# zju3dv/street_gaussians

Hardware: AMD Instinct MI355X
Metric: train iters/s (fwd+bwd) @1M Gaussians 1920x1280 SH3 (higher is better)
Workload: dtype f32

## Files before the change

### street_gaussians_amd/csrc/sgr_blend_bwd.hip

```cpp
#include "sgr_math.h"
#include "sgr_reduce.h"

#include <type_traits>

#ifndef SGR_WITH_VARIANTS
#define SGR_WITH_VARIANTS 0
#endif

#define SGR_TILE_THREADS 256
typedef float sgr_f2 __attribute__((ext_vector_type(2)));
#ifndef SGR_BWD_BATCH
#define SGR_BWD_BATCH 128
#endif
#ifndef SGR_BWD_BATCH_WIDE
#define SGR_BWD_BATCH_WIDE 64
#endif
#ifndef SGR_BWD_WAVES
#define SGR_BWD_WAVES(SMAX) ((SMAX) >= 12 && (SMAX) <= 16 ? 6 : ((SMAX) >= 20 && (SMAX) <= 24 ? 5 : ((SMAX) > 24 ? 4 : 1)))
#endif
template <int SMAX>
struct SgrBwdBatch { static constexpr int value = SMAX <= 8 ? SGR_BWD_BATCH : SGR_BWD_BATCH_WIDE; };
#define SGR_ROW_BASE 11
#ifndef SGR_FACTORED
#define SGR_FACTORED 1
#endif
#ifndef SGR_EXACT_BWD_FAST
#define SGR_EXACT_BWD_FAST 1
#endif
#ifndef SGR_BWD_NEWTON
#define SGR_BWD_NEWTON 0
#endif
#ifndef SGR_EXACT_BWD_GUARD
#define SGR_EXACT_BWD_GUARD 1
#endif
#ifndef SGR_EXACT_TRIM
#define SGR_EXACT_TRIM 1
#endif
#ifndef SGR_FOLD
#define SGR_FOLD 1
#endif
#ifndef SGR_VROWS
#define SGR_VROWS 1
#endif
#ifndef SGR_SPARSE_K
#define SGR_SPARSE_K 9
#endif

__global__ void sgr_wave_sum_test_kernel(const float* in, float* out_dpp, float* out_shfl) {
    const float v = in[blockIdx.x * 64 + threadIdx.x];
    float a = v, a1 = 2.f * v, a2 = -v, a3 = v + 1.f;
    sgr_wave_sum4(a, a1, a2, a3);
    const float b = sgr_wave_sum_shfl(v);
    const float c = sgr_wave_sum_dpp(v);
    float x[12], r[3];
#pragma unroll
    for (int i = 0; i < 12; i++) x[i] = (float)(i + 1) * v;
    sgr_wave_reduce_scatter<12>(x, r);
    const int k = threadIdx.x >> 4;
    const int perm = (k == 1) ? 2 : ((k == 2) ? 1 : k);
    bool rs_ok = true;
#pragma unroll
    for (int t = 0; t < 3; t++) rs_ok = rs_ok && (r[t] == (float)(4 * t + perm + 1) * b);
    {
        float y[12], g[1];
#pragma unroll
        for (int i = 0; i < 12; i++) y[i] = (float)(i + 1) * v;
        sgr_wave_reduce_fold<12>(y, g);
        const int bank = (threadIdx.x >> 2) & 3, t0 = (0x3120 >> (bank * 4)) & 3;
        if (t0 < 3) rs_ok = rs_ok && (g[0] == (float)(4 * t0 + perm + 1) * b);
        float z[32], gz[2];
#pragma unroll
        for (int i = 0; i < 32; i++) z[i] = (float)(i + 1) * v;
        sgr_wave_reduce_fold<32>(z, gz);
#pragma unroll
        for (int i = 0; i < 2; i++) rs_ok = rs_ok && (gz[i] == (float)(4 * (4 * i + t0) + perm + 1) * b);
        float w[20], gw[2];
#pragma unroll
        for (int i = 0; i < 20; i++) w[i] = (float)(i + 1) * v;
        sgr_wave_reduce_fold<20>(w, gw);
#pragma unroll
        for (int i = 0; i < 2; i++)
            if (4 * i + t0 < 5) rs_ok = rs_ok && (gw[i] == (float)(4 * (4 * i + t0) + perm + 1) * b);
    }
    {
        float z[24], g0, g1;
#pragma unroll
        for (int i = 0; i < 24; i++) z[i] = (float)(i + 1) * v;
        sgr_wave_reduce_fold24(z, g0, g1);
        const int bank = (threadIdx.x >> 2) & 3, pb = (0x3120 >> (bank * 4)) & 3;
        rs_ok = rs_ok && (g0 == (float)(4 * pb + perm + 1) * b);
        if ((bank & 1) == 0) rs_ok = rs_ok && (g1 == (float)(16 + 4 * pb + perm + 1) * b);
    }
    rs_ok = __all(rs_ok);
    if (threadIdx.x == 63) {
        const bool ok = (a1 == 2.f * a) && (a2 == -a) && (a3 == a + 64.f) && (c == a) && rs_ok;
        out_dpp[blockIdx.x] = ok ? a : __builtin_nanf("");
        out_shfl[blockIdx.x] = b;
    }
}
void sgr_launch_wave_sum_test(const float* in, float* out_dpp, float* out_shfl, int nwaves, hipStream_t s) {
    sgr_wave_sum_test_kernel<<<nwaves, 64, 0, s>>>(in, out_dpp, out_shfl);
}

__device__ __forceinline__ void sgr_lds_barrier() {
    asm volatile("s_waitcnt lgkmcnt(0)" ::: "memory");
    __syncthreads();
}

__device__ __forceinline__ uint32_t sgr_lds_addr(const float* p) {
    return (uint32_t)(uintptr_t)(__attribute__((address_space(3))) const float*)p;
}
__device__ __forceinline__ int sgr_popc64(uint64_t m) {
    int r;
    asm("s_bcnt1_i32_b64 %0, %1" : "=s"(r) : "s"(m) : "scc");
    return r;
}

template <int SMAX, bool CULL, bool DPP, bool DET, int BATCH, bool EXACT = false>
__device__ __forceinline__ void
sgr_blend_bwd_body(const uint2* __restrict__ ranges, const uint32_t* __restrict__ point_list, int W, int H, int S,
                     int gx, int gy, const float* __restrict__ bg_color, const float4* __restrict__ rec,
                     const uint32_t* __restrict__ u0, const uint64_t* __restrict__ tmask, const float* __restrict__ semantics, const float* __restrict__ alphas,
                     const uint32_t* __restrict__ n_contrib, const uint8_t* __restrict__ hit4,
                     const float* __restrict__ dL_dpixels, const float* __restrict__ dL_dpixel_depths,
                     const float* __restrict__ dL_dalphas, const float* __restrict__ dL_dpixel_semantics,
                     float* __restrict__ partials, int row_stride, uint8_t* __restrict__ touched, uint32_t row_limit,
                     const uint32_t* __restrict__ hlist, const uint32_t* __restrict__ n_contrib_k, const uint32_t* __restrict__ hl_flag) {
#pragma clang fp contract(off)
    constexpr int NS = SMAX > 0 ? SMAX : 1;
    constexpr int NVAL = (SGR_ROW_BASE + SMAX + 3) / 4 * 4;
    constexpr int ACCW = NVAL + (((NVAL / 4) & 1) ? 0 : 4);
    __shared__ float4 sA[BATCH];
    __shared__ float4 sB[BATCH];
    __shared__ float4 sC[BATCH];
    __shared__ uint64_t sBits[4][4];
    __shared__ uint64_t sVis[4][4];
    __shared__ int sMax[4];
    constexpr int NROW = DET ? 2 : 1;
    constexpr bool VROWS = SGR_VROWS && DET && DPP && SGR_FOLD && SMAX == 0;
    constexpr int CAP = NROW * BATCH;
    constexpr int NCH = BATCH / 64;
    constexpr int SPK = (VROWS && SMAX == 0) ? SGR_SPARSE_K : 0;
    constexpr int XROWS = 4 * SPK;
    static_assert(SPK == 0 || ACCW == 12, "a stage entry is a row of 12 floats");
    static_assert(SPK <= 16, "add sparse cases");
    __shared__ __attribute__((aligned(16))) float sAcc[(CAP + XROWS) * ACCW];
    __shared__ __attribute__((aligned(16))) float sSem[SMAX > 0 ? BATCH * SMAX : 4];

    const int tid = threadIdx.x, lane = tid & 63, wave = tid >> 6;
    uint32_t tx, ty;
    if (!sgr_wg_tile(blockIdx.x, gx, gy, ranges, tx, ty)) return;
    const uint32_t tile = ty * (uint32_t)gx + tx;
    const uint32_t px = tx * SGR_BLOCK_X + (wave & 1) * 8 + (lane & 7);
    const uint32_t py = ty * SGR_BLOCK_Y + (wave >> 1) * 8 + (lane >> 3);
    const bool inside = px < (uint32_t)W && py < (uint32_t)H;
    const float pxf = (float)px, pyf = (float)py;
    const size_t pix_id = (size_t)W * py + px;
    const size_t plane = (size_t)H * W;
    const uint2 range = ranges[tile];

    const float T_final = inside ? (1.0f - alphas[pix_id]) : 0.0f;
    float T = T_final;
    const bool HL = SGR_HLIST && CULL && hit4 != nullptr && hlist != nullptr && hl_flag[0] != 0u;
    const int lastc = inside ? (int)(HL ? n_contrib_k : n_contrib)[pix_id] : 0;
    float dLdC0 = 0.f, dLdC1 = 0.f, dLdC2 = 0.f, dLdD = 0.f, dLdA = 0.f;
    float dLdS[NS];
#pragma unroll
    for (int i = 0; i < NS; i++) dLdS[i] = 0.f;
    if (inside) {
        dLdC0 = dL_dpixels[pix_id];
        dLdC1 = dL_dpixels[plane + pix_id];
        dLdC2 = dL_dpixels[2 * plane + pix_id];
        dLdD = dL_dpixel_depths[pix_id];
        dLdA = dL_dalphas[pix_id];
        if (SMAX > 0) {
#pragma unroll
            for (int i = 0; i < SMAX; i++)
                if (i < S) dLdS[i] = dL_dpixel_semantics[i * plane + pix_id];
        }
    }
    const float bgdot = bg_color[0] * dLdC0 + bg_color[1] * dLdC1 + bg_color[2] * dLdC2;
    const bool bg_zero = bg_color[0] == 0.0f && bg_color[1] == 0.0f && bg_color[2] == 0.0f;
    constexpr float LSC = EXACT ? 1.0f : SGR_LOG2E;
    const float kx = (0.5f * (float)W) / LSC, ky = (0.5f * (float)H) / LSC;

    sgr_f2 acc01 = {0.f, 0.f}, acc2D = {0.f, 0.f}, last01 = {0.f, 0.f}, last2D = {0.f, 0.f};
    const sgr_f2 dL01 = {dLdC0, dLdC1}, dL2D = {dLdC2, dLdD};
    float accA = 0.f, last_alpha = 0.f;
    constexpr int NREC = SGR_FACTORED ? 1 : NS;
    float accS[NREC], lastS[NREC];
#pragma unroll
    for (int i = 0; i < NREC; i++) { accS[i] = 0.f; lastS[i] = 0.f; }
    float Arec = 0.f, u_last = 0.f;

    int mx = lastc;
#pragma unroll
    for (int o = 32; o >= 1; o >>= 1) mx = max(mx, __shfl_xor(mx, o, 64));
    if (lane == 0) sMax[wave] = mx;
    sgr_lds_barrier();
    const int maxc = max(max(sMax[0], sMax[1]), max(sMax[2], sMax[3]));
    const float tx0 = (float)(tx * SGR_BLOCK_X), ty0 = (float)(ty * SGR_BLOCK_Y);
    const int acc_lane_off = (DET ? (wave >> 1) : 0) * BATCH * ACCW + (lane >> 4);
    const int fold_t0 = (0x3120 >> (((lane >> 2) & 3) * 4)) & 3;
    const bool fold_leader = (lane & 3) == 0;
    const int acc_fold_off = (VROWS ? 0 : (DET ? (wave >> 1) : 0) * BATCH * ACCW) + 4 * fold_t0 + (lane >> 4);
    const int wave_s = __builtin_amdgcn_readfirstlane(wave);

#ifndef SGR_BWD_PREFETCH
#define SGR_BWD_PREFETCH 1
#endif
    auto entry = [&](const int k) __attribute__((always_inline)) -> uint32_t {
        return HL ? hlist[range.x + (uint32_t)k] : (uint32_t)k;
    };
    uint32_t g_pre = 0, h_pre = 0;
    if (SGR_BWD_PREFETCH) {
        const int pos0 = (tid < BATCH) ? (maxc - 1) - tid : -1;
        if (pos0 >= 0) {
            const uint32_t lp = entry(pos0);
            g_pre = point_list[range.x + lp];
            if (CULL && hit4 != nullptr) h_pre = hit4[range.x + lp];
        }
    }
    for (int hi = maxc - 1; hi >= 0;) {
        sgr_lds_barrier();
        const bool stager = tid < BATCH;
        const int pos = stager ? hi - tid : -1;
        uint32_t mask4 = 0;
        if (!VROWS) {
#pragma unroll
            for (int row = tid; row < NROW * BATCH; row += SGR_TILE_THREADS) {
                float4* z = reinterpret_cast<float4*>(&sAcc[row * ACCW]);
#pragma unroll
                for (int k4 = 0; k4 < ACCW / 4; k4++) z[k4] = make_float4(0.f, 0.f, 0.f, 0.f);
            }
        }
        const uint32_t g_raw = pos >= 0 ? (SGR_BWD_PREFETCH ? g_pre : point_list[range.x + entry(pos)]) : SGR_DEAD;
        const uint32_t h_raw = (pos >= 0 && CULL && hit4 != nullptr) ? (SGR_BWD_PREFETCH ? h_pre : (uint32_t)hit4[range.x + entry(pos)]) : 0xFu;
        if (pos >= 0 && !(g_raw & SGR_DEAD) && h_raw != 0u) {
            const uint32_t g = g_raw;
            const float4* r = rec + 4 * (size_t)g;
            const float4 a = r[0];
            const float4 b = r[1];
            const float4 d4 = r[3];
            sB[tid] = EXACT ? make_float4(-0.5f * b.x, -b.y, -0.5f * b.z, b.w)
                            : sgr_stage_conic(b);
            sC[tid] = r[2];
            const uint32_t dy_ = __float_as_uint(d4.y);
            const uint32_t urow = sgr_row_of(dy_, tx, ty, u0, tmask, g);
            sA[tid] = make_float4(a.x, a.y, __uint_as_float(urow), 0.0f);
            if (SMAX > 0) {
#pragma unroll
                for (int ch = 0; ch < SMAX; ch++) sSem[tid * SMAX + ch] = ch < S ? semantics[(size_t)g * S + ch] : 0.0f;
            }
            mask4 = CULL ? (hit4 != nullptr ? h_raw : sgr_quadrant_mask(a, b, tx0, ty0)) : 0xFu;
            if (urow >= row_limit) mask4 = 0;
        }
        if (SGR_BWD_PREFETCH) {
            const int posn = stager ? (hi - BATCH) - tid : -1;
            if (posn >= 0) {
                const uint32_t lp = entry(posn);
                g_pre = point_list[range.x + lp];
                if (CULL && hit4 != nullptr) h_pre = hit4[range.x + lp];
            }
        }
        if (stager) {
#pragma unroll
            for (int q = 0; q < 4; q++) {
                const uint64_t m = __ballot((mask4 >> q) & 1u);
                if (lane == 0) sBits[q][wave] = m;
            }
        }
        sgr_lds_barrier();

        int lim = BATCH;
        uint64_t vm[4][NCH];
        int vfirst[4] = {0, 0, 0, 0};
        if constexpr (VROWS) {
            auto below = [](const uint64_t m, const int nb) { return nb >= 64 ? m : (nb <= 0 ? 0ull : (m & ((1ull << nb) - 1ull))); };
            uint64_t raw[4][NCH];
            int total = 0;
#pragma unroll
            for (int q = 0; q < 4; q++)
#pragma unroll
                for (int c = 0; c < NCH; c++) {
                    raw[q][c] = sgr_uniform_u64(sBits[q][c]);
                    total += sgr_popc64(raw[q][c]);
                }
            if (total > CAP) {
                for (lim = BATCH - 32; lim > 32; lim -= 32) {
                    int t = 0;
#pragma unroll
                    for (int q = 0; q < 4; q++)
#pragma unroll
                        for (int c = 0; c < NCH; c++) t += sgr_popc64(below(raw[q][c], lim - 64 * c));
                    if (t <= CAP) break;
                }
            }
            int first = 0;
#pragma unroll
            for (int q = 0; q < 4; q++) {
                vfirst[q] = first;
#pragma unroll
                for (int c = 0; c < NCH; c++) {
                    vm[q][c] = below(raw[q][c], lim - 64 * c);
                    first += sgr_popc64(vm[q][c]);
                }
            }
        }
        int rown = 0;
        constexpr int kq = SPK;
        const int stage_off = (CAP + wave_s * SPK) * ACCW;
        if constexpr (VROWS) {
#pragma unroll
            for (int q = 0; q < 4; q++) rown = (wave_s == q) ? vfirst[q] : rown;
        }
        (void)kq; (void)stage_off;

        uint64_t vis = 0;
        auto process = [&](const int j, const float4 q, const float dx, const float dy, const float power2, const float G,
                           const float alpha) __attribute__((always_inline)) {
                const int posj = hi - j;
                const bool k0 = posj < lastc, k1 = !(power2 > 0.0f), k2 = !(alpha < SGR_ALPHA_MIN);
                const uint64_t hm = __builtin_amdgcn_ballot_w64(k0) & __builtin_amdgcn_ballot_w64(k1) &
                                    __builtin_amdgcn_ballot_w64(k2);
                if (hm == 0) return;
                const int rowi = rown;
                if constexpr (VROWS) {
                    rown++;
                    vis = sgr_bitset1(vis, j & 63);
                }
                const bool hit = k0 && k1 && k2;

                const float4 c = sC[j];
                float v[NVAL];
#pragma unroll
                for (int k = 0; k < NVAL; k++) v[k] = 0.0f;
                float Gd = 0.0f, wm = 0.0f;
                if (hit) {
                    const float oma = 1.0f - alpha;
                    float inv1ma = __builtin_amdgcn_rcpf(oma);
                    if (SGR_BWD_NEWTON || (EXACT && !SGR_EXACT_BWD_FAST))
                        inv1ma = fmaf(fmaf(-oma, inv1ma, 1.0f), inv1ma, inv1ma);
                    T = (EXACT && !SGR_EXACT_BWD_FAST) ? (SGR_EXACT_TRIM ? sgr_div_by(T, oma, inv1ma) : T / oma) : T * inv1ma;
                    wm = alpha * T;
                    const float one_m_la = 1.0f - last_alpha;
                    float d;
                    if (SGR_FACTORED) {
                        Arec = fmaf(last_alpha, u_last, one_m_la * Arec);
                        float u = fmaf(c.x, dLdC0, dLdA);
                        u = fmaf(c.y, dLdC1, u);
                        u = fmaf(c.z, dLdC2, u);
                        u = fmaf(c.w, dLdD, u);
                        if (SMAX > 0) {
                            const float4* sj = reinterpret_cast<const float4*>(&sSem[j * SMAX]);
#pragma unroll
                            for (int c4 = 0; c4 < SMAX / 4; c4++) {
                                const float4 s4 = sj[c4];
                                u = fmaf(s4.x, dLdS[4 * c4], u);
                                u = fmaf(s4.y, dLdS[4 * c4 + 1], u);
                                u = fmaf(s4.z, dLdS[4 * c4 + 2], u);
                                u = fmaf(s4.w, dLdS[4 * c4 + 3], u);
                            }
                        }
                        d = u - Arec;
                        u_last = u;
                    } else {
                    const sgr_f2 c01 = {c.x, c.y}, c2D = {c.z, c.w};
                    const sgr_f2 la2 = {last_alpha, last_alpha};
                    acc01 = __builtin_elementwise_fma(la2, last01, one_m_la * acc01);
                    acc2D = __builtin_elementwise_fma(la2, last2D, one_m_la * acc2D);
                    const sgr_f2 t = __builtin_elementwise_fma(c2D - acc2D, dL2D, (c01 - acc01) * dL01);
                    d = t.x + t.y;
                    accA = fmaf(one_m_la, accA, last_alpha);
                    d = fmaf(1.0f - accA, dLdA, d);
                    if (SMAX > 0) {
                        const float4* sj = reinterpret_cast<const float4*>(&sSem[j * SMAX]);
#pragma unroll
                        for (int c4 = 0; c4 < SMAX / 4; c4++) {
                            const float4 s4 = sj[c4];
                            const float svv[4] = {s4.x, s4.y, s4.z, s4.w};
#pragma unroll
                            for (int e = 0; e < 4; e++) {
                                const int ch = (4 * c4 + e) % NREC;
                                accS[ch] = fmaf(last_alpha, lastS[ch], one_m_la * accS[ch]);
                                d = fmaf(svv[e] - accS[ch], dLdS[4 * c4 + e], d);
                                lastS[ch] = svv[e];
                            }
                        }
                    }
                    last01 = c01;
                    last2D = c2D;
                    }
                    last_alpha = alpha;
                    d *= T;
                    if (EXACT && SGR_EXACT_BWD_FAST)
                        Gd = bg_zero ? G * d : G * (d + (-T_final * inv1ma) * bgdot);
                    else if (EXACT)
                        Gd = (SGR_EXACT_TRIM && bg_zero) ? G * d
                                                         : G * (d + (SGR_EXACT_TRIM ? sgr_div_by(-T_final, oma, inv1ma) : -T_final / oma) * bgdot);
                    else
                        Gd = G * fmaf(-T_final * inv1ma, bgdot, d);
                }
                if (SMAX > 0 && !(DPP && SGR_FOLD)) {
#pragma unroll
                    for (int ch = 0; ch < SMAX; ch++) v[SGR_ROW_BASE + ch] = wm * dLdS[ch];
                }
                const float gx = Gd * dx, gy = Gd * dy;
                float ax, ay;
                {
#pragma clang fp contract(off)
                    const float e1 = fmaf(q.y, dy, q.x * dx), e2 = q.z * dy;
                    ax = fmaf(q.x, dx, e1);
                    ay = fmaf(q.y, dx, e2 + e2);
                }
                v[0] = gx;
                v[1] = gy;
                v[2] = fabsf(Gd) * fmaf(fabsf(ax), kx, fabsf(ay) * ky);
                v[3] = gx * dx;
                v[4] = gx * dy;
                v[5] = gy * dy;
                v[6] = Gd;
                const sgr_f2 o01 = wm * dL01, o2D = wm * dL2D;
                v[7] = o01.x;
                v[8] = o01.y;
                v[9] = o2D.x;
                v[10] = o2D.y;
                float r[NVAL / 4];
                if constexpr (SPK > 0) {
                    const int kc = sgr_popc64(hm);
                    if (kc <= kq) {
                        if (hit) {
                            const uint32_t rank = __builtin_amdgcn_mbcnt_hi((uint32_t)(hm >> 32), __builtin_amdgcn_mbcnt_lo((uint32_t)hm, 0u));
                            const uint32_t ea = sgr_lds_addr(sAcc + stage_off) + rank * 48u;
#define SGR_STAGE_ST(OFF, VAL) asm volatile("ds_write_b32 %0, %1 offset:" #OFF : : "v"(ea), "v"(VAL) : "memory")
                            SGR_STAGE_ST(0, v[0]); SGR_STAGE_ST(4, v[2]); SGR_STAGE_ST(8, v[1]); SGR_STAGE_ST(12, v[3]);
                            SGR_STAGE_ST(16, v[4]); SGR_STAGE_ST(20, v[6]); SGR_STAGE_ST(24, v[5]); SGR_STAGE_ST(28, v[7]);
                            SGR_STAGE_ST(32, v[8]); SGR_STAGE_ST(36, v[10]); SGR_STAGE_ST(40, v[9]); SGR_STAGE_ST(44, v[11]);
#undef SGR_STAGE_ST
                        }
                        __builtin_amdgcn_wave_barrier();
                        if (fold_leader && fold_t0 < NVAL / 4) {
                            const float* src = sAcc + (acc_fold_off + stage_off);
                            auto sum_first = [&](auto KC) __attribute__((always_inline)) {
                                constexpr int kk = decltype(KC)::value, k0 = kk < 8 ? kk : 8;
                                float a[k0];
#pragma unroll
                                for (int e = 0; e < k0; e++) a[e] = src[e * 12];
                                float t = a[0];
#pragma unroll
                                for (int e = 1; e < k0; e++) t += a[e];
                                if constexpr (kk > 8) {
                                    float b[kk - 8];
#pragma unroll
                                    for (int e = 8; e < kk; e++) b[e - 8] = src[e * 12];
#pragma unroll
                                    for (int e = 8; e < kk; e++) t += b[e - 8];
                                }
                                return t;
                            };
                            float t = 0.0f;
                            switch (kc) {
#define SGR_SPARSE_CASE(N) case N: if constexpr (N <= SPK) t = sum_first(std::integral_constant<int, (N <= SPK ? N : 1)>{}); break
                                SGR_SPARSE_CASE(1); SGR_SPARSE_CASE(2); SGR_SPARSE_CASE(3); SGR_SPARSE_CASE(4);
                                SGR_SPARSE_CASE(5); SGR_SPARSE_CASE(6); SGR_SPARSE_CASE(7); SGR_SPARSE_CASE(8);
                                SGR_SPARSE_CASE(9); SGR_SPARSE_CASE(10); SGR_SPARSE_CASE(11); SGR_SPARSE_CASE(12);
                                SGR_SPARSE_CASE(13); SGR_SPARSE_CASE(14); SGR_SPARSE_CASE(15); SGR_SPARSE_CASE(16);
#undef SGR_SPARSE_CASE
                                default: break;
                            }
                            sAcc[acc_fold_off + rowi * ACCW] = t;
                            asm volatile("; sparse visit done" ::: "memory");
                        }
                        return;
                    }
                }
                if (DPP && SGR_FOLD) {
                    float* dst = sAcc + (acc_fold_off + (VROWS ? rowi : j) * ACCW);
                    auto fold_chunk = [&](auto C0, auto CN) __attribute__((always_inline)) {
                        constexpr int c0 = decltype(C0)::value, cn = decltype(CN)::value;
                        float vv[cn], g[1];
#pragma unroll
                        for (int k = 0; k < cn; k++) {
                            const int idx = c0 + k;
                            vv[k] = idx < SGR_ROW_BASE ? v[idx < NVAL ? idx : 0]
                                                       : (idx - SGR_ROW_BASE < SMAX ? wm * dLdS[(idx - SGR_ROW_BASE) % NS] : 0.0f);
                        }
                        sgr_wave_reduce_fold<cn>(vv, g);
                        if (fold_leader && fold_t0 < cn / 4) {
                            if constexpr (VROWS) dst[c0] = g[0];
                            else atomicAdd(&dst[c0], g[0]);
                        }
                    };
                    fold_chunk(std::integral_constant<int, 0>{}, std::integral_constant<int, (NVAL < 16 ? NVAL : 16)>{});
                    if constexpr (NVAL > 16)
                        fold_chunk(std::integral_constant<int, 16>{}, std::integral_constant<int, (NVAL - 16 < 16 ? NVAL - 16 : 16)>{});
                    if constexpr (NVAL > 32)
                        fold_chunk(std::integral_constant<int, 32>{}, std::integral_constant<int, (NVAL - 32 < 16 ? NVAL - 32 : 16)>{});
                    static_assert(NVAL <= 48, "add a fold chunk");
                    return;
                } else if (DPP) {
                    sgr_wave_reduce_scatter<NVAL>(v, r);
                } else {
#pragma unroll
                    for (int t = 0; t < NVAL / 4; t++) {
                        const float s0 = sgr_wave_sum_shfl(v[4 * t]), s1 = sgr_wave_sum_shfl(v[4 * t + 1]);
                        const float s2 = sgr_wave_sum_shfl(v[4 * t + 2]), s3 = sgr_wave_sum_shfl(v[4 * t + 3]);
                        const int k = lane >> 4;
                        r[t] = k == 0 ? s0 : (k == 1 ? s2 : (k == 2 ? s1 : s3));
                    }
                }
                if ((lane & 15) == 0) {
                    const int k = lane >> 4;
                    float* dst = sAcc + (acc_lane_off + j * ACCW);
                    (void)k;
#pragma unroll
                    for (int t = 0; t < NVAL / 4; t++) atomicAdd(&dst[4 * t], r[t]);
                }
        };
        auto exactG = [&](const float pw, const float opac) __attribute__((always_inline)) -> float {
            if constexpr (SGR_EXACT_BWD_FAST != 0) {
                float g = __builtin_amdgcn_exp2f(pw * SGR_LOG2E);
                const bool near = fabsf(opac * g - SGR_ALPHA_MIN) <= 4.0e-6f * SGR_ALPHA_MIN;
                if (SGR_EXACT_BWD_GUARD && __builtin_amdgcn_ballot_w64(near) != 0) g = SGR_EXACT_TRIM ? sgr_expf_ref(pw) : expf(pw);
                return g;
            } else {
                return SGR_EXACT_TRIM ? sgr_expf_ref(pw) : expf(pw);
            }
        };
        for (int chunk = 0; chunk < BATCH / 64; chunk++) {
            uint64_t m;
            m = sBits[wave][chunk];
            m = sgr_uniform_u64(m);
            if constexpr (VROWS) {
                const int nb = lim - 64 * chunk;
                m = nb >= 64 ? m : (nb <= 0 ? 0ull : (m & ((1ull << nb) - 1ull)));
            }
            if (__builtin_popcountll(m) & 1) {
                const int j0 = chunk * 64 + sgr_pop_lowest(m);
                const float4 a0 = sA[j0], q0 = sB[j0];
                const float dx0 = a0.x - pxf, dy0 = a0.y - pyf;
                const float pw0 = EXACT ? sgr_power_ref_staged(q0.x, q0.y, q0.z, dx0, dy0) : sgr_power2(q0.x, q0.y, q0.z, dx0, dy0);
                const float G0 = EXACT ? exactG(pw0, q0.w) : __builtin_amdgcn_exp2f(pw0);
                process(j0, q0, dx0, dy0, pw0, G0, fminf(0.99f, q0.w * G0));
            }
            while (m) {
                const int j0 = chunk * 64 + sgr_pop_lowest(m);
                const int j1 = chunk * 64 + sgr_pop_lowest(m);
                const float4 a0 = sA[j0], q0 = sB[j0];
                const float4 a1 = sA[j1], q1 = sB[j1];
                const float dx0 = a0.x - pxf, dy0 = a0.y - pyf, dx1 = a1.x - pxf, dy1 = a1.y - pyf;
                const float pw0 = EXACT ? sgr_power_ref_staged(q0.x, q0.y, q0.z, dx0, dy0) : sgr_power2(q0.x, q0.y, q0.z, dx0, dy0);
                const float pw1 = EXACT ? sgr_power_ref_staged(q1.x, q1.y, q1.z, dx1, dy1) : sgr_power2(q1.x, q1.y, q1.z, dx1, dy1);
                const float G0 = EXACT ? exactG(pw0, q0.w) : __builtin_amdgcn_exp2f(pw0), G1 = EXACT ? exactG(pw1, q1.w) : __builtin_amdgcn_exp2f(pw1);
                const float al0 = fminf(0.99f, q0.w * G0), al1 = fminf(0.99f, q1.w * G1);
                process(j0, q0, dx0, dy0, pw0, G0, al0);
                process(j1, q1, dx1, dy1, pw1, G1, al1);
            }
            if constexpr (VROWS) {
                if (lane == 0) sVis[wave][chunk] = vis;
                vis = 0;
            }
        }
        sgr_lds_barrier();
        uint64_t vq[4][NCH];
        if constexpr (VROWS) {
#pragma unroll
            for (int q = 0; q < 4; q++)
#pragma unroll
                for (int c = 0; c < NCH; c++) vq[q][c] = sgr_uniform_u64(sVis[q][c]);
        }
        if (mask4 != 0 && tid < lim) {
            const uint32_t u = __float_as_uint(sA[tid].z);
            touched[u] = 1;
            float4* row = reinterpret_cast<float4*>(partials + (size_t)u * row_stride);
            float4 r[NVAL / 4];
#pragma unroll
            for (int k4 = 0; k4 < NVAL / 4; k4++) r[k4] = make_float4(0.f, 0.f, 0.f, 0.f);
            if constexpr (VROWS) {
#pragma unroll
                for (int q = 0; q < 4; q++) {
                    int before = vfirst[q];
#pragma unroll
                    for (int c = 0; c + 1 < NCH; c++) before += (c < wave_s) ? sgr_popc64(vq[q][c]) : 0;
                    uint64_t mine = vq[q][0];
#pragma unroll
                    for (int c = 1; c < NCH; c++) mine = (wave_s == c) ? vq[q][c] : mine;
                    if ((mine >> lane) & 1ull) {
                        const int rq = before + (int)__builtin_amdgcn_mbcnt_hi((uint32_t)(mine >> 32), __builtin_amdgcn_mbcnt_lo((uint32_t)mine, 0u));
                        const float4* src = reinterpret_cast<const float4*>(&sAcc[rq * ACCW]);
#pragma unroll
                        for (int k4 = 0; k4 < NVAL / 4; k4++) {
                            const float4 t = src[k4];
                            r[k4].x += t.x; r[k4].y += t.y; r[k4].z += t.z; r[k4].w += t.w;
                        }
                    }
                }
            } else {
                const float4* src = reinterpret_cast<const float4*>(&sAcc[tid * ACCW]);
#pragma unroll
                for (int k4 = 0; k4 < NVAL / 4; k4++) r[k4] = src[k4];
                if (DET) {
                    const float4* src1 = reinterpret_cast<const float4*>(&sAcc[(BATCH + tid) * ACCW]);
#pragma unroll
                    for (int k4 = 0; k4 < NVAL / 4; k4++) {
                        const float4 t = src1[k4];
                        r[k4].x += t.x; r[k4].y += t.y; r[k4].z += t.z; r[k4].w += t.w;
                    }
                }
            }
            {
                const float4 qq = sB[tid];
                const float sgx = r[0].x, sgy = r[0].z, qw = qq.w, hq = -0.5f * qq.w;
                r[0].x = qw * kx * fmaf(qq.x + qq.x, sgx, qq.y * sgy);
                r[0].z = qw * ky * fmaf(qq.z + qq.z, sgy, qq.y * sgx);
                r[0].y = qw * r[0].y;
                r[0].w = hq * r[0].w;
                r[1].x = hq * r[1].x;
                r[1].z = hq * r[1].z;
            }
#pragma unroll
            for (int k4 = 0; k4 < NVAL / 4; k4++) row[k4] = make_float4(r[k4].x, r[k4].z, r[k4].y, r[k4].w);
        }
        hi -= lim;
        if (SGR_BWD_PREFETCH && lim != BATCH) {
            const int posn = stager ? hi - tid : -1;
            if (posn >= 0) {
                const uint32_t lp = entry(posn);
                g_pre = point_list[range.x + lp];
                if (CULL && hit4 != nullptr) h_pre = hit4[range.x + lp];
            }
        }
    }
}

#define SGR_BWD_ARGS                                                                                                  \
    const uint2 *__restrict__ ranges, const uint32_t *__restrict__ point_list, int W, int H, int S, int gx, int gy,       \
        const float *__restrict__ bg_color, const float4 *__restrict__ rec, const uint32_t *__restrict__ u0, const uint64_t *__restrict__ tmask,          \
        const float *__restrict__ semantics,          \
        const float *__restrict__ alphas, const uint32_t *__restrict__ n_contrib, const uint8_t *__restrict__ hit4,        \
        const float *__restrict__ dL_dpixels, const float *__restrict__ dL_dpixel_depths,                                  \
        const float *__restrict__ dL_dalphas,                                                                              \
        const float *__restrict__ dL_dpixel_semantics, float *__restrict__ partials, int row_stride,                      \
        uint8_t *__restrict__ touched, uint32_t row_limit, const uint32_t *__restrict__ hlist,  \
        const uint32_t *__restrict__ n_contrib_k, const uint32_t *__restrict__ hl_flag
#define SGR_BWD_PASS                                                                                                  \
    ranges, point_list, W, H, S, gx, gy, bg_color, rec, u0, tmask, semantics, alphas, n_contrib, hit4, dL_dpixels,               \
        dL_dpixel_depths, dL_dalphas, dL_dpixel_semantics, partials, row_stride, touched, row_limit, hlist, n_contrib_k, hl_flag
template <int SMAX, bool CULL, bool DPP, bool DET>
__global__ void __launch_bounds__(SGR_TILE_THREADS) __attribute__((amdgpu_waves_per_eu(SGR_BWD_WAVES(SMAX))))
sgr_blend_bwd_kernel(SGR_BWD_ARGS) {
    sgr_blend_bwd_body<SMAX, CULL, DPP, DET, SgrBwdBatch<SMAX>::value>(SGR_BWD_PASS);
}
template <bool CULL, bool DPP, bool DET>
__global__ void __launch_bounds__(SGR_TILE_THREADS) __attribute__((amdgpu_waves_per_eu(8, 8)))
sgr_blend_bwd_kernel_s0(SGR_BWD_ARGS) {
    sgr_blend_bwd_body<0, CULL, DPP, DET, SgrBwdBatch<0>::value>(SGR_BWD_PASS);
}
#ifndef SGR_BWD_EXACT_WAVES
#define SGR_BWD_EXACT_WAVES(SMAX) ((SMAX) == 0 ? 8 : SGR_BWD_WAVES(SMAX))
#endif
template <int SMAX>
__global__ void __launch_bounds__(SGR_TILE_THREADS) __attribute__((amdgpu_waves_per_eu(SGR_BWD_EXACT_WAVES(SMAX))))
sgr_blend_bwd_kernel_exact(SGR_BWD_ARGS) {
    sgr_blend_bwd_body<SMAX, true, true, true, SgrBwdBatch<SMAX>::value, true>(SGR_BWD_PASS);
}

#if SGR_WITH_VARIANTS
#define SGR_V2_BATCH 64
#define SGR_V2_CH 8
#ifndef SGR_V2_WAVES
#define SGR_V2_WAVES 5
#endif
template <bool CULL, bool DET>
__global__ void __launch_bounds__(SGR_TILE_THREADS) __attribute__((amdgpu_waves_per_eu(SGR_V2_WAVES, SGR_V2_WAVES)))
sgr_blend_bwd_kernel_v2(SGR_BWD_ARGS) {
#pragma clang fp contract(off)
    constexpr int BATCH = SGR_V2_BATCH, CH = SGR_V2_CH, ACCW = 12, NROW = DET ? 2 : 1;
    __shared__ float4 sA[BATCH];
    __shared__ float4 sB[BATCH];
    __shared__ float4 sC[BATCH];
    __shared__ uint32_t sU[BATCH];
    __shared__ uint32_t sFlag[BATCH];
    __shared__ uint64_t sBits[4];
    __shared__ int sMax[4];
    __shared__ __attribute__((aligned(16))) float sAcc[NROW * BATCH * ACCW];
    __shared__ __attribute__((aligned(16))) float2 sW[4][CH][64];
    __shared__ float4 sDL[4][64];
    __shared__ int sVis[4][CH];
    (void)S; (void)semantics; (void)dL_dpixel_semantics;

    const int tid = threadIdx.x, lane = tid & 63, wave = tid >> 6;
    uint32_t tx, ty;
    if (!sgr_wg_tile(blockIdx.x, gx, gy, ranges, tx, ty)) return;
    const uint32_t tile = ty * (uint32_t)gx + tx;
    const uint32_t qx0 = tx * SGR_BLOCK_X + (wave & 1) * 8, qy0 = ty * SGR_BLOCK_Y + (wave >> 1) * 8;
    const uint32_t px = qx0 + (lane & 7), py = qy0 + (lane >> 3);
    const bool inside = px < (uint32_t)W && py < (uint32_t)H;
    const float pxf = (float)px, pyf = (float)py;
    const size_t pix_id = (size_t)W * py + px;
    const size_t plane = (size_t)H * W;
    const uint2 range = ranges[tile];

    const float T_final = inside ? (1.0f - alphas[pix_id]) : 0.0f;
    float T = T_final;
    const int lastc = inside ? (int)n_contrib[pix_id] : 0;
    float dLdC0 = 0.f, dLdC1 = 0.f, dLdC2 = 0.f, dLdD = 0.f, dLdA = 0.f;
    if (inside) {
        dLdC0 = dL_dpixels[pix_id];
        dLdC1 = dL_dpixels[plane + pix_id];
        dLdC2 = dL_dpixels[2 * plane + pix_id];
        dLdD = dL_dpixel_depths[pix_id];
        dLdA = dL_dalphas[pix_id];
    }
    sDL[wave][lane] = make_float4(dLdC0, dLdC1, dLdC2, dLdD);
    const float bgdot = bg_color[0] * dLdC0 + bg_color[1] * dLdC1 + bg_color[2] * dLdC2;
    const float kx = (0.5f * (float)W) / SGR_LOG2E, ky = (0.5f * (float)H) / SGR_LOG2E;

    float Arec = 0.f, u_last = 0.f, last_alpha = 0.f;

    int mx = lastc;
#pragma unroll
    for (int o = 32; o >= 1; o >>= 1) mx = max(mx, __shfl_xor(mx, o, 64));
    if (lane == 0) sMax[wave] = mx;
    sgr_lds_barrier();
    const int maxc = max(max(sMax[0], sMax[1]), max(sMax[2], sMax[3]));
    const float tx0 = (float)(tx * SGR_BLOCK_X), ty0 = (float)(ty * SGR_BLOCK_Y);
    const int pv = lane >> 3, pg = lane & 7;
    const float bpx = (float)(qx0 + (uint32_t)pg), bpy0 = (float)qy0;
    const int rowset = (DET ? (wave >> 1) : 0) * BATCH * ACCW;

    for (int hi = maxc - 1; hi >= 0; hi -= BATCH) {
        sgr_lds_barrier();
        const bool stager = tid < BATCH;
        const int pos = stager ? hi - tid : -1;
        uint32_t mask4 = 0;
        if (stager) sFlag[tid] = 0;
        if (tid < NROW * BATCH) {
            float4* z = reinterpret_cast<float4*>(&sAcc[tid * ACCW]);
            z[0] = make_float4(0.f, 0.f, 0.f, 0.f);
            z[1] = make_float4(0.f, 0.f, 0.f, 0.f);
            z[2] = make_float4(0.f, 0.f, 0.f, 0.f);
        }
        if (pos >= 0) {
            const uint32_t g = point_list[range.x + (uint32_t)pos] & ~SGR_DEAD;
            const float4* r = rec + 4 * (size_t)g;
            const float4 a = r[0];
            const float4 b = r[1];
            const float4 d4 = r[3];
            sA[tid] = a;
            sB[tid] = sgr_stage_conic(b);
            sC[tid] = r[2];
            const uint32_t dy_ = __float_as_uint(d4.y);
            sU[tid] = sgr_row_of(dy_, tx, ty, u0, tmask, g);
            mask4 = CULL ? (hit4 != nullptr ? (uint32_t)hit4[range.x + (uint32_t)pos] : sgr_quadrant_mask(a, b, tx0, ty0))
                         : 0xFu;
        }
        if (stager) {
#pragma unroll
            for (int q = 0; q < 4; q++) {
                const uint64_t m = __ballot((mask4 >> q) & 1u);
                if (lane == 0) sBits[q] = m;
            }
        }
        sgr_lds_barrier();

        auto pass_a = [&](const int j, const int c, const float4 q, const float dx, const float dy, const float power2,
                          const float G, const float alpha) __attribute__((always_inline)) {
            (void)dx; (void)dy;
            const int posj = hi - j;
            const bool hit = (posj < lastc) && !(power2 > 0.0f) && !(alpha < SGR_ALPHA_MIN);
            float Gd = 0.0f, wm = 0.0f;
            if (hit) {
                const float4 cc = sC[j];
                const float oma = 1.0f - alpha;
                float inv1ma = __builtin_amdgcn_rcpf(oma);
                inv1ma = fmaf(fmaf(-oma, inv1ma, 1.0f), inv1ma, inv1ma);
                T = T * inv1ma;
                wm = alpha * T;
                const float one_m_la = 1.0f - last_alpha;
                float u = fmaf(cc.x, dLdC0, dLdA);
                u = fmaf(cc.y, dLdC1, u);
                u = fmaf(cc.z, dLdC2, u);
                u = fmaf(cc.w, dLdD, u);
                Arec = fmaf(last_alpha, u_last, one_m_la * Arec);
                float d = u - Arec;
                u_last = u;
                last_alpha = alpha;
                d *= T;
                const float dopa = fmaf(-T_final * inv1ma, bgdot, d);
                Gd = G * dopa;
            }
            (void)q;
            sW[wave][c][lane ^ ((c & 3) << 3)] = make_float2(Gd, wm);
            if (lane == 0) sVis[wave][c] = j;
        };

        auto pass_b = [&](const int nv) __attribute__((always_inline)) {
            float m0 = 0.f, m1x = 0.f, m1y = 0.f, m2xx = 0.f, m2xy = 0.f, m2yy = 0.f, wabs = 0.f;
            float c0 = 0.f, c1 = 0.f, c2 = 0.f, cD = 0.f;
            const bool act = pv < nv;
            int j = 0;
            float4 q = make_float4(0.f, 0.f, 0.f, 0.f);
            if (act) {
                j = sVis[wave][pv];
                const float4 a = sA[j];
                q = sB[j];
                const float dx = a.x - bpx;
                const float qa2 = q.x + q.x, qc2 = q.z + q.z;
                const float qbdx = q.y * dx;
                const int swz = (pv & 3) << 3;
#pragma unroll
                for (int i = 0; i < 8; i++) {
                    const int p = 8 * i + pg;
                    const float2 wv = sW[wave][pv][p ^ swz];
                    const float4 dl = sDL[wave][p];
                    const float dy = a.y - (bpy0 + (float)i);
                    const float Gd = wv.x, wmv = wv.y;
                    const float gxx = Gd * dx, gyy = Gd * dy;
                    m0 += Gd;
                    m1x += gxx;
                    m1y += gyy;
                    m2xx = fmaf(gxx, dx, m2xx);
                    m2xy = fmaf(gxx, dy, m2xy);
                    m2yy = fmaf(gyy, dy, m2yy);
                    const float A = fmaf(qa2, dx, q.y * dy), B = fmaf(qc2, dy, qbdx);
                    wabs = fmaf(fabsf(Gd), fmaf(fabsf(A), kx, fabsf(B) * ky), wabs);
                    c0 = fmaf(wmv, dl.x, c0);
                    c1 = fmaf(wmv, dl.y, c1);
                    c2 = fmaf(wmv, dl.z, c2);
                    cD = fmaf(wmv, dl.w, cD);
                }
            }
            sgr_fold4(m0, wabs);
            sgr_fold4(m1x, c0);
            sgr_fold4(m1y, c1);
            sgr_fold4(m2xx, c2);
            sgr_fold4(m2xy, cD);
            sgr_half4(m2yy);
            sgr_quad_sum2(m0, m1x);
            sgr_quad_sum2(m1y, m2xx);
            sgr_quad_sum2(m2xy, m2yy);
            if (act && (lane & 3) == 0) {
                const bool odd = (lane >> 2) & 1;
                const float qw = q.w;
                const float e0 = qw * kx * fmaf(q.x + q.x, m1x, q.y * m1y);
                const float e1 = qw * ky * fmaf(q.z + q.z, m1y, q.y * m1x);
                const float h = -0.5f * qw;
                float* dst = sAcc + (rowset + j * ACCW);
                atomicAdd(&dst[odd ? 2 : 0], odd ? qw * m0 : e0);
                atomicAdd(&dst[odd ? 7 : 1], odd ? m1x : e1);
                atomicAdd(&dst[odd ? 8 : 3], odd ? m1y : h * m2xx);
                atomicAdd(&dst[odd ? 9 : 4], odd ? m2xx : h * m2xy);
                atomicAdd(&dst[odd ? 10 : 5], odd ? m2xy : h * m2yy);
                if (!odd) {
                    atomicAdd(&dst[6], m0);
                    sFlag[j] = 1u;
                }
            }
        };

        uint64_t m = sgr_uniform_u64(sBits[wave]);
        while (m) {
            int nv = 0;
            for (int trip = 0; trip < CH / 2 && m; trip++) {
                const int j0 = __ffsll((unsigned long long)m) - 1;
                m &= m - 1;
                const bool two = m != 0;
                const int j1 = two ? (__ffsll((unsigned long long)m) - 1) : j0;
                m &= m - 1;
                const float4 a0 = sA[j0], q0 = sB[j0];
                const float4 a1 = sA[j1], q1 = sB[j1];
                const float dx0 = a0.x - pxf, dy0 = a0.y - pyf, dx1 = a1.x - pxf, dy1 = a1.y - pyf;
                const float pw0 = sgr_power2(q0.x, q0.y, q0.z, dx0, dy0);
                const float pw1 = sgr_power2(q1.x, q1.y, q1.z, dx1, dy1);
                const float G0 = __builtin_amdgcn_exp2f(pw0), G1 = __builtin_amdgcn_exp2f(pw1);
                const float al0 = fminf(0.99f, q0.w * G0), al1 = fminf(0.99f, q1.w * G1);
                pass_a(j0, nv, q0, dx0, dy0, pw0, G0, al0);
                nv++;
                if (two) {
                    pass_a(j1, nv, q1, dx1, dy1, pw1, G1, al1);
                    nv++;
                }
            }
            __builtin_amdgcn_wave_barrier();
            pass_b(nv);
            __builtin_amdgcn_wave_barrier();
        }
        sgr_lds_barrier();
        const uint32_t flags = stager ? sFlag[tid] : 0u;
        if (flags) {
            const uint32_t u = sU[tid];
            touched[u] = 1;
            float4* row = reinterpret_cast<float4*>(partials + (size_t)u * row_stride);
            const float4* src = reinterpret_cast<const float4*>(&sAcc[tid * ACCW]);
            float4 r0 = src[0], r1 = src[1], r2 = src[2];
            if (DET) {
// ... 100 lines not shown
```

### street_gaussians_amd/csrc/sgr_reduce.h

```cpp
#pragma once
#include <hip/hip_runtime.h>

__device__ __forceinline__ float sgr_wave_sum_dpp(float v) {
#define SGR_DPP_ADD(ctrl, rmask)                                                                              \
    v += __builtin_bit_cast(float, __builtin_amdgcn_update_dpp(0, __builtin_bit_cast(int, v), ctrl, rmask, 0xF, false))
    SGR_DPP_ADD(0xB1, 0xF);
    SGR_DPP_ADD(0x4E, 0xF);
    SGR_DPP_ADD(0x141, 0xF);
    SGR_DPP_ADD(0x140, 0xF);
    SGR_DPP_ADD(0x142, 0xA);
    SGR_DPP_ADD(0x143, 0xC);
#undef SGR_DPP_ADD
    return v;
}

__device__ __forceinline__ float sgr_wave_sum_shfl(float v) {
#pragma unroll
    for (int o = 32; o >= 1; o >>= 1) v += __shfl_xor(v, o, 64);
    return v;
}

template <bool DPP>
__device__ __forceinline__ float sgr_wave_sum(float v) {
    return DPP ? sgr_wave_sum_dpp(v) : sgr_wave_sum_shfl(v);
}

#define SGR_DPP4(ctrl)                                                                             \
    "v_add_f32_dpp %0, %0, %0 " ctrl "\n\tv_add_f32_dpp %1, %1, %1 " ctrl "\n\tv_add_f32_dpp %2, %2, %2 " ctrl \
    "\n\tv_add_f32_dpp %3, %3, %3 " ctrl "\n\t"
__device__ __forceinline__ void sgr_wave_sum4(float& a, float& b, float& c, float& d) {
    asm volatile("s_nop 1\n\t" SGR_DPP4("quad_perm:[1,0,3,2] row_mask:0xf bank_mask:0xf")
                 SGR_DPP4("quad_perm:[2,3,0,1] row_mask:0xf bank_mask:0xf")
                 SGR_DPP4("row_half_mirror row_mask:0xf bank_mask:0xf")
                 SGR_DPP4("row_mirror row_mask:0xf bank_mask:0xf")
                 SGR_DPP4("row_bcast:15 row_mask:0xa bank_mask:0xf")
                 SGR_DPP4("row_bcast:31 row_mask:0xc bank_mask:0xf") "s_nop 0"
                 : "+v"(a), "+v"(b), "+v"(c), "+v"(d));
}
#undef SGR_DPP4

__device__ __forceinline__ void sgr_swap32(float& a, float& b) {
    auto r = __builtin_amdgcn_permlane32_swap(__builtin_bit_cast(unsigned, a), __builtin_bit_cast(unsigned, b), false, false);
    a = __builtin_bit_cast(float, (unsigned)r[0]);
    b = __builtin_bit_cast(float, (unsigned)r[1]);
}
__device__ __forceinline__ void sgr_swap16(float& a, float& b) {
    auto r = __builtin_amdgcn_permlane16_swap(__builtin_bit_cast(unsigned, a), __builtin_bit_cast(unsigned, b), false, false);
    a = __builtin_bit_cast(float, (unsigned)r[0]);
    b = __builtin_bit_cast(float, (unsigned)r[1]);
}
#define SGR_ROW4(ctrl)                                                                              \
    "v_add_f32_dpp %0, %0, %0 " ctrl "\n\tv_add_f32_dpp %1, %1, %1 " ctrl "\n\tv_add_f32_dpp %2, %2, %2 " ctrl \
    "\n\tv_add_f32_dpp %3, %3, %3 " ctrl "\n\t"
#define SGR_ROW3(ctrl)                                                                              \
    "v_add_f32_dpp %0, %0, %0 " ctrl "\n\tv_add_f32_dpp %1, %1, %1 " ctrl "\n\tv_add_f32_dpp %2, %2, %2 " ctrl "\n\t"
#define SGR_ROW2(ctrl) "v_add_f32_dpp %0, %0, %0 " ctrl "\n\tv_add_f32_dpp %1, %1, %1 " ctrl "\n\ts_nop 0\n\t"
#define SGR_ROWSTEPS(M)                                                                                        \
    "s_nop 1\n\t" M("quad_perm:[1,0,3,2] row_mask:0xf bank_mask:0xf") M("quad_perm:[2,3,0,1] row_mask:0xf bank_mask:0xf") \
        M("row_half_mirror row_mask:0xf bank_mask:0xf") M("row_mirror row_mask:0xf bank_mask:0xf") "s_nop 0"
__device__ __forceinline__ void sgr_row_sum4(float& a, float& b, float& c, float& d) {
    asm volatile(SGR_ROWSTEPS(SGR_ROW4) : "+v"(a), "+v"(b), "+v"(c), "+v"(d));
}
__device__ __forceinline__ void sgr_row_sum3(float& a, float& b, float& c) {
    asm volatile(SGR_ROWSTEPS(SGR_ROW3) : "+v"(a), "+v"(b), "+v"(c));
}
__device__ __forceinline__ void sgr_row_sum2(float& a, float& b) { asm volatile(SGR_ROWSTEPS(SGR_ROW2) : "+v"(a), "+v"(b)); }
#undef SGR_ROW4
#undef SGR_ROW3
#undef SGR_ROW2
#undef SGR_ROWSTEPS

template <int NVAL>
__device__ __forceinline__ void sgr_wave_reduce_scatter(float (&v)[NVAL], float (&r)[NVAL / 4]) {
    static_assert(NVAL % 4 == 0, "pad the value count to a multiple of 4");
    float h[NVAL / 2];
#pragma unroll
    for (int p = 0; p < NVAL / 2; p++) {
        sgr_swap32(v[2 * p], v[2 * p + 1]);
        h[p] = v[2 * p] + v[2 * p + 1];
    }
#pragma unroll
    for (int t = 0; t < NVAL / 4; t++) {
        sgr_swap16(h[2 * t], h[2 * t + 1]);
        r[t] = h[2 * t] + h[2 * t + 1];
    }
    constexpr int N = NVAL / 4;
    int t = 0;
#pragma unroll
    for (; t + 4 <= N && (N - t) != 5; t += 4) sgr_row_sum4(r[t], r[t + 1], r[t + 2], r[t + 3]);
#pragma unroll
    for (; t + 3 <= N; t += 3) sgr_row_sum3(r[t], r[t + 1], r[t + 2]);
    if (t + 2 == N) sgr_row_sum2(r[t], r[t + 1]);
    static_assert(N != 1, "unsupported value count");
}

__device__ __forceinline__ void sgr_fold8(float& a, const float b) {
    asm volatile("s_nop 1\n\tv_add_f32_dpp %0, %0, %0 row_ror:8 row_mask:0xf bank_mask:0x3\n\t"
                 "v_add_f32_dpp %0, %1, %1 row_ror:8 row_mask:0xf bank_mask:0xc"
                 : "+v"(a)
                 : "v"(b));
}
__device__ __forceinline__ void sgr_self8(float& a) {
    asm volatile("s_nop 1\n\tv_add_f32_dpp %0, %0, %0 row_ror:8 row_mask:0xf bank_mask:0xf" : "+v"(a));
}
__device__ __forceinline__ void sgr_fold4(float& a, const float b) {
    asm volatile("s_nop 1\n\tv_add_f32_dpp %0, %0, %0 row_shl:4 row_mask:0xf bank_mask:0x5\n\t"
                 "v_add_f32_dpp %0, %1, %1 row_shr:4 row_mask:0xf bank_mask:0xa"
                 : "+v"(a)
                 : "v"(b));
}
__device__ __forceinline__ void sgr_half4(float& a) {
    asm volatile("s_nop 1\n\tv_add_f32_dpp %0, %0, %0 row_shl:4 row_mask:0xf bank_mask:0x5" : "+v"(a));
}
__device__ __forceinline__ void sgr_quad_sum(float& a) {
    asm volatile("s_nop 1\n\tv_add_f32_dpp %0, %0, %0 quad_perm:[2,3,0,1] row_mask:0xf bank_mask:0xf\n\ts_nop 1\n\t"
                 "v_add_f32_dpp %0, %0, %0 quad_perm:[1,0,3,2] row_mask:0xf bank_mask:0xf\n\ts_nop 0"
                 : "+v"(a));
}
__device__ __forceinline__ void sgr_quad_sum2(float& a, float& b) {
    asm volatile("s_nop 1\n\tv_add_f32_dpp %0, %0, %0 quad_perm:[2,3,0,1] row_mask:0xf bank_mask:0xf\n\t"
                 "v_add_f32_dpp %1, %1, %1 quad_perm:[2,3,0,1] row_mask:0xf bank_mask:0xf\n\ts_nop 0\n\t"
                 "v_add_f32_dpp %0, %0, %0 quad_perm:[1,0,3,2] row_mask:0xf bank_mask:0xf\n\t"
                 "v_add_f32_dpp %1, %1, %1 quad_perm:[1,0,3,2] row_mask:0xf bank_mask:0xf\n\ts_nop 0"
                 : "+v"(a), "+v"(b));
}
template <int NVAL>
__device__ __forceinline__ void sgr_wave_reduce_fold(float (&v)[NVAL], float (&g)[(NVAL / 4 + 3) / 4]) {
    static_assert(NVAL % 4 == 0, "pad the value count to a multiple of 4");
    constexpr int N = NVAL / 4, NF = (N + 1) / 2, NG = (NF + 1) / 2;
    float h[NVAL / 2], r[N];
#pragma unroll
    for (int p = 0; p < NVAL / 2; p++) {
        sgr_swap32(v[2 * p], v[2 * p + 1]);
        h[p] = v[2 * p] + v[2 * p + 1];
    }
#pragma unroll
    for (int t = 0; t < N; t++) {
        sgr_swap16(h[2 * t], h[2 * t + 1]);
        r[t] = h[2 * t] + h[2 * t + 1];
    }
#pragma unroll
    for (int i = 0; i < N / 2; i++) sgr_fold8(r[2 * i], r[2 * i + 1]);
    if (N & 1) sgr_self8(r[N - 1]);
#pragma unroll
    for (int i = 0; i < NG; i++) {
        if (2 * i + 1 < NF) sgr_fold4(r[4 * i], r[4 * i + 2 < N ? 4 * i + 2 : N - 1]);
        else sgr_half4(r[4 * i]);
        g[i] = r[4 * i];
    }
    int i = 0;
#pragma unroll
    for (; i + 2 <= NG; i += 2) sgr_quad_sum2(g[i], g[i + 1]);
    if (i < NG) sgr_quad_sum(g[i]);
}


__device__ __forceinline__ void sgr_wave_reduce_fold24(float (&v)[24], float& g0, float& g1) {
    float h[12], r[6];
#pragma unroll
    for (int p = 0; p < 12; p++) {
        sgr_swap32(v[2 * p], v[2 * p + 1]);
        h[p] = v[2 * p] + v[2 * p + 1];
    }
#pragma unroll
    for (int t = 0; t < 6; t++) {
        sgr_swap16(h[2 * t], h[2 * t + 1]);
        r[t] = h[2 * t] + h[2 * t + 1];
    }
#define SGR_RM " row_mask:0xf bank_mask:"
    asm volatile(
        "s_nop 1\n\t"
        "v_add_f32_dpp %0, %0, %0 row_ror:8" SGR_RM "0x3\n\t"
        "v_add_f32_dpp %2, %2, %2 row_ror:8" SGR_RM "0x3\n\t"
        "v_add_f32_dpp %4, %4, %4 row_ror:8" SGR_RM "0x3\n\t"
        "v_add_f32_dpp %0, %1, %1 row_ror:8" SGR_RM "0xc\n\t"
        "v_add_f32_dpp %2, %3, %3 row_ror:8" SGR_RM "0xc\n\t"
        "v_add_f32_dpp %4, %5, %5 row_ror:8" SGR_RM "0xc\n\t"
        "v_add_f32_dpp %0, %0, %0 row_shl:4" SGR_RM "0x5\n\t"
        "v_add_f32_dpp %0, %2, %2 row_shr:4" SGR_RM "0xa\n\t"
        "v_add_f32_dpp %4, %4, %4 row_shl:4" SGR_RM "0x5\n\t"
        "s_nop 0\n\t"
        "v_add_f32_dpp %0, %0, %0 quad_perm:[2,3,0,1]" SGR_RM "0xf\n\t"
        "v_add_f32_dpp %4, %4, %4 quad_perm:[2,3,0,1]" SGR_RM "0xf\n\t"
        "s_nop 0\n\t"
        "v_add_f32_dpp %0, %0, %0 quad_perm:[1,0,3,2]" SGR_RM "0xf\n\t"
        "v_add_f32_dpp %4, %4, %4 quad_perm:[1,0,3,2]" SGR_RM "0xf\n\t"
        "s_nop 0"
        : "+v"(r[0]), "+v"(r[1]), "+v"(r[2]), "+v"(r[3]), "+v"(r[4]), "+v"(r[5]));
#undef SGR_RM
    g0 = r[0];
    g1 = r[4];
}
```

Baseline: 635.8.

## Reduce separable pixel-offset moments instead of per-pixel gradient products in blend backward

Adds a separable-moment path (SGR_SEPMOM, on by default) for the VROWS backward variant. Instead of reducing per-pixel products like gx*dx, each wave reduces Gd-weighted moments in wave-centred pixel offsets, 8 values instead of 12, with a new DPP fold that builds the X and X² moments from the partial sums. The per-Gaussian gradient terms are then rebuilt from these moments and the Gaussian mean during the final row accumulation. This cuts cross-lane reduction work and register pressure in the hot backward loop, at the cost of a more involved reconstruction and a different floating-point summation order.

```diff
diff --git a/street_gaussians_amd/csrc/sgr_blend_bwd.hip b/street_gaussians_amd/csrc/sgr_blend_bwd.hip
--- a/street_gaussians_amd/csrc/sgr_blend_bwd.hip
+++ b/street_gaussians_amd/csrc/sgr_blend_bwd.hip
@@ -44,6 +44,9 @@
 #endif
 #ifndef SGR_SPARSE_K
 #define SGR_SPARSE_K 9
+#endif
+#ifndef SGR_SEPMOM
+#define SGR_SEPMOM 1
 #endif
 
 __global__ void sgr_wave_sum_test_kernel(const float* in, float* out_dpp, float* out_shfl) {
@@ -90,6 +93,17 @@
         const int bank = (threadIdx.x >> 2) & 3, pb = (0x3120 >> (bank * 4)) & 3;
         rs_ok = rs_ok && (g0 == (float)(4 * pb + perm + 1) * b);
         if ((bank & 1) == 0) rs_ok = rs_ok && (g1 == (float)(16 + 4 * pb + perm + 1) * b);
+    }
+    {
+        float s[8], g0, g1;
+#pragma unroll
+        for (int i = 0; i < 8; i++) s[i] = (float)(i + 1) * v;
+        const float X = (float)(threadIdx.x & 7) - 3.5f;
+        sgr_wave_reduce_sep8(s, X, g0, g1);
+        const float bx = sgr_wave_sum_shfl(v * X), bxx = sgr_wave_sum_shfl(v * (X * X));
+        const int bank = (threadIdx.x >> 2) & 3, i = 4 * (bank >> 1) + perm;
+        if (bank & 1) rs_ok = rs_ok && (g0 == (float)(i + 1) * bx);
+        else rs_ok = rs_ok && (g0 == (float)(i + 1) * b) && (g1 == (float)(i + 1) * bxx);
     }
     rs_ok = __all(rs_ok);
     if (threadIdx.x == 63) {
@@ -144,6 +158,7 @@
     constexpr int XROWS = 4 * SPK;
     static_assert(SPK == 0 || ACCW == 12, "a stage entry is a row of 12 floats");
     static_assert(SPK <= 16, "add sparse cases");
+    constexpr bool SEP = SGR_SEPMOM && VROWS;
     __shared__ __attribute__((aligned(16))) float sAcc[(CAP + XROWS) * ACCW];
     __shared__ __attribute__((aligned(16))) float sSem[SMAX > 0 ? BATCH * SMAX : 4];
 
@@ -205,6 +220,16 @@
     const bool fold_leader = (lane & 3) == 0;
     const int acc_fold_off = (VROWS ? 0 : (DET ? (wave >> 1) : 0) * BATCH * ACCW) + 4 * fold_t0 + (lane >> 4);
     const int wave_s = __builtin_amdgcn_readfirstlane(wave);
+    const float sep_cx = tx0 + (float)((wave_s & 1) * 8) + 3.5f, sep_cy = ty0 + (float)((wave_s >> 1) * 8) + 3.5f;
+    const float sepX = pxf - sep_cx, sepY = pyf - sep_cy;
+    int sep_pos = -1;
+    {
+        const int bank = (lane >> 2) & 3, i = 4 * (bank >> 1) + ((0x3120 >> ((lane >> 4) * 4)) & 3);
+        if ((lane & 3) == 0) sep_pos = (bank & 1) ? (i == 0 ? 1 : (i == 1 ? 4 : -1)) : (int)((0xA9876520u >> (4 * i)) & 0xFu);
+        if ((lane & 3) == 1 && bank == 0 && i == 0) sep_pos = 3;
+    }
+    const bool sep_g1 = (lane & 3) == 1;
+    (void)sep_pos; (void)sep_g1;
 
 #ifndef SGR_BWD_PREFETCH
 #define SGR_BWD_PREFETCH 1
@@ -433,9 +458,16 @@
                             const uint32_t rank = __builtin_amdgcn_mbcnt_hi((uint32_t)(hm >> 32), __builtin_amdgcn_mbcnt_lo((uint32_t)hm, 0u));
                             const uint32_t ea = sgr_lds_addr(sAcc + stage_off) + rank * 48u;
 #define SGR_STAGE_ST(OFF, VAL) asm volatile("ds_write_b32 %0, %1 offset:" #OFF : : "v"(ea), "v"(VAL) : "memory")
-                            SGR_STAGE_ST(0, v[0]); SGR_STAGE_ST(4, v[2]); SGR_STAGE_ST(8, v[1]); SGR_STAGE_ST(12, v[3]);
-                            SGR_STAGE_ST(16, v[4]); SGR_STAGE_ST(20, v[6]); SGR_STAGE_ST(24, v[5]); SGR_STAGE_ST(28, v[7]);
-                            SGR_STAGE_ST(32, v[8]); SGR_STAGE_ST(36, v[10]); SGR_STAGE_ST(40, v[9]); SGR_STAGE_ST(44, v[11]);
+                            if constexpr (SEP) {
+                                const float gX = Gd * sepX, gY = Gd * sepY;
+                                SGR_STAGE_ST(0, v[6]); SGR_STAGE_ST(4, gX); SGR_STAGE_ST(8, gY); SGR_STAGE_ST(12, gX * sepX);
+                                SGR_STAGE_ST(16, gY * sepX); SGR_STAGE_ST(20, gY * sepY); SGR_STAGE_ST(24, v[2]); SGR_STAGE_ST(28, v[7]);
+                                SGR_STAGE_ST(32, v[8]); SGR_STAGE_ST(36, v[9]); SGR_STAGE_ST(40, v[10]); SGR_STAGE_ST(44, v[11]);
+                            } else {
+                                SGR_STAGE_ST(0, v[0]); SGR_STAGE_ST(4, v[2]); SGR_STAGE_ST(8, v[1]); SGR_STAGE_ST(12, v[3]);
+                                SGR_STAGE_ST(16, v[4]); SGR_STAGE_ST(20, v[6]); SGR_STAGE_ST(24, v[5]); SGR_STAGE_ST(28, v[7]);
+                                SGR_STAGE_ST(32, v[8]); SGR_STAGE_ST(36, v[10]); SGR_STAGE_ST(40, v[9]); SGR_STAGE_ST(44, v[11]);
+                            }
 #undef SGR_STAGE_ST
                         }
                         __builtin_amdgcn_wave_barrier();
@@ -473,6 +505,13 @@
                         }
                         return;
                     }
+                }
+                if constexpr (SEP) {
+                    const float gY = Gd * sepY;
+                    float s8[8] = {Gd, gY, gY * sepY, v[2], v[7], v[8], v[9], v[10]}, g0, g1;
+                    sgr_wave_reduce_sep8(s8, sepX, g0, g1);
+                    if (sep_pos >= 0) sAcc[rowi * ACCW + sep_pos] = sep_g1 ? g1 : g0;
+                    return;
                 }
                 if (DPP && SGR_FOLD) {
                     float* dst = sAcc + (acc_fold_off + (VROWS ? rowi : j) * ACCW);
@@ -576,6 +615,11 @@
             float4 r[NVAL / 4];
 #pragma unroll
             for (int k4 = 0; k4 < NVAL / 4; k4++) r[k4] = make_float4(0.f, 0.f, 0.f, 0.f);
+            sgr_f2 mrel = {0.f, 0.f};
+            if constexpr (SEP) {
+                const float4 mean = sA[tid];
+                mrel = sgr_f2{mean.x - tx0, mean.y - ty0};
+            }
             if constexpr (VROWS) {
 #pragma unroll
                 for (int q = 0; q < 4; q++) {
@@ -588,10 +632,27 @@
                     if ((mine >> lane) & 1ull) {
                         const int rq = before + (int)__builtin_amdgcn_mbcnt_hi((uint32_t)(mine >> 32), __builtin_amdgcn_mbcnt_lo((uint32_t)mine, 0u));
                         const float4* src = reinterpret_cast<const float4*>(&sAcc[rq * ACCW]);
-#pragma unroll
-                        for (int k4 = 0; k4 < NVAL / 4; k4++) {
-                            const float4 t = src[k4];
-                            r[k4].x += t.x; r[k4].y += t.y; r[k4].z += t.z; r[k4].w += t.w;
+                        if constexpr (SEP) {
+                            const float4 t0 = src[0], t1 = src[1], t2 = src[2];
+                            const float a = mrel.x - (float)((q & 1) * 8 + 3.5f), b = mrel.y - (float)((q >> 1) * 8 + 3.5f);
+                            const float s0 = t0.x, sx = t0.y, sy = t0.z;
+                            r[0].x += fmaf(a, s0, -sx);
+                            r[0].z += fmaf(b, s0, -sy);
+                            r[0].w += fmaf(a, fmaf(a, s0, -2.0f * sx), t0.w);
+                            r[1].x += fmaf(a, fmaf(b, s0, -sy), fmaf(-b, sx, t1.x));
+                            r[1].z += fmaf(b, fmaf(b, s0, -2.0f * sy), t1.y);
+                            r[0].y += t1.z;
+                            r[1].y += s0;
+                            r[1].w += t1.w;
+                            r[2].x += t2.x;
+                            r[2].z += t2.y;
+                            r[2].y += t2.z;
+                        } else {
+#pragma unroll
+                            for (int k4 = 0; k4 < NVAL / 4; k4++) {
+                                const float4 t = src[k4];
+                                r[k4].x += t.x; r[k4].y += t.y; r[k4].z += t.z; r[k4].w += t.w;
+                            }
                         }
                     }
                 }
diff --git a/street_gaussians_amd/csrc/sgr_reduce.h b/street_gaussians_amd/csrc/sgr_reduce.h
--- a/street_gaussians_amd/csrc/sgr_reduce.h
+++ b/street_gaussians_amd/csrc/sgr_reduce.h
@@ -154,6 +154,39 @@
     if (i < NG) sgr_quad_sum(g[i]);
 }
 
+__device__ __forceinline__ void sgr_wave_reduce_sep8(float (&v)[8], const float X, float& g0, float& g1) {
+    float h[4], r[2];
+#pragma unroll
+    for (int p = 0; p < 4; p++) {
+        sgr_swap32(v[2 * p], v[2 * p + 1]);
+        h[p] = v[2 * p] + v[2 * p + 1];
+    }
+#pragma unroll
+    for (int t = 0; t < 2; t++) {
+        sgr_swap16(h[2 * t], h[2 * t + 1]);
+        r[t] = h[2 * t] + h[2 * t + 1];
+    }
+    sgr_fold8(r[0], r[1]);
+    g0 = r[0];
+    const float vx = g0 * X;
+    g1 = vx * X;
+#define SGR_RM " row_mask:0xf bank_mask:"
+    asm volatile(
+        "s_nop 1\n\t"
+        "v_add_f32_dpp %0, %0, %0 row_shl:4" SGR_RM "0x5\n\t"
+        "v_add_f32_dpp %1, %1, %1 row_shl:4" SGR_RM "0x5\n\t"
+        "v_add_f32_dpp %0, %2, %2 row_shr:4" SGR_RM "0xa\n\t"
+        "s_nop 1\n\t"
+        "v_add_f32_dpp %1, %1, %1 quad_perm:[2,3,0,1]" SGR_RM "0xf\n\t"
+        "v_add_f32_dpp %0, %0, %0 quad_perm:[2,3,0,1]" SGR_RM "0xf\n\t"
+        "s_nop 0\n\t"
+        "v_add_f32_dpp %1, %1, %1 quad_perm:[1,0,3,2]" SGR_RM "0xf\n\t"
+        "v_add_f32_dpp %0, %0, %0 quad_perm:[1,0,3,2]" SGR_RM "0xf\n\t"
+        "s_nop 0"
+        : "+v"(g0), "+v"(g1)
+        : "v"(vx));
+#undef SGR_RM
+}
 
 __device__ __forceinline__ void sgr_wave_reduce_fold24(float (&v)[24], float& g0, float& g1) {
     float h[12], r[6];
```

Result: faster. 651.0 (median of 6 runs) (+2.4%).
